# Lymphatus/caesium-clt

Measured on AMD Instinct MI355X. Metric: megapixels/sec JPEG q=80 1920x1080 batch, higher is better.
Workload: dtype int32

## Files before the change

### caesium-clt_amd/csrc/k_trellis.hip

```cpp
#include <algorithm>
#include <atomic>
#include <cassert>
#include <utility>

#include "kernels.h"

namespace csh {

#define CSH_TR_CAP 16
#define CSH_TR_WGU uint32_t(CSH_TR_WG)
#define CSH_TR_SPILL (63 - CSH_TR_CAP)
#define CSH_TR_MAXWG 2048
size_t trellis_spill_words(uint32_t nslots) { return size_t(nslots) * CSH_TR_SPILL * 3u * CSH_TR_WGU; }

#ifdef CSH_EMUL
#define CSH_ANY(p) (p)
#define CSH_WAVE_OR(v) (v)
#define CSH_SPILL_LD(ptr) (*(ptr))
#define CSH_SPILL_ST(ptr, v) (*(ptr) = (v))
#else
#define CSH_ANY(p) (__ballot(p) != 0ull)
__device__ __forceinline__ static unsigned tr_wave_or(unsigned v) {
    const unsigned n = 32u - unsigned(__clz(v));
    unsigned r = 0;
    if (__ballot(n >= 8u)) r = 8u;
    if (__ballot(n >= r + 4u)) r += 4u;
    if (__ballot(n >= r + 2u)) r += 2u;
    if (__ballot(n >= r + 1u)) r += 1u;
    return r ? 1u << (r - 1u) : 0u;
}
#define CSH_WAVE_OR(v) tr_wave_or(v)
#define CSH_SPILL_LD(ptr) __builtin_nontemporal_load(ptr)
#define CSH_SPILL_ST(ptr, v) __builtin_nontemporal_store((v), (ptr))
#endif

using Oct8 = std::integer_sequence<int, 0, 1, 2, 3, 4, 5, 6, 7>;
static constexpr uint8_t kN2Z[64] = {0,  1,  5,  6,  14, 15, 27, 28, 2,  4,  7,  13, 16, 26, 29, 42, 3,  8,  12, 17, 25, 30,
                                     41, 43, 9,  11, 18, 24, 31, 40, 44, 53, 10, 19, 23, 32, 39, 45, 52, 54, 20, 22, 33, 38,
                                     46, 51, 55, 60, 21, 34, 37, 47, 50, 56, 59, 61, 35, 36, 48, 49, 57, 58, 62, 63};
template <int I>
__device__ __forceinline__ static int tr_half(const uint4 &v) {
    uint32_t w = (I / 2 == 0) ? v.x : (I / 2 == 1) ? v.y : (I / 2 == 2) ? v.z : v.w;
    return (I & 1) ? (int(w) >> 16) : (int(w << 16) >> 16);
}
template <int J, int... I>
__device__ __forceinline__ static void tr_unpack(int r[64], const uint4 &v, std::integer_sequence<int, I...>) { ((r[8 * J + I] = tr_half<I>(v)), ...); }
template <int... J>
__device__ __forceinline__ static void tr_load(const int16_t *__restrict__ blk, int r[64], std::integer_sequence<int, J...>) {
    const uint4 v[8] = {*reinterpret_cast<const uint4 *>(blk + CSH_RAW_OCT * J)...};
    (tr_unpack<J>(r, v[J], Oct8()), ...);
}
__device__ __forceinline__ static int tr_level(int x, int d, uint32_t mul, uint32_t sh) {
    const uint32_t a = uint32_t(x + (d >> 1)) << sh;
    return int(uint32_t((uint64_t(a & 0xFFFFFFu) * uint64_t(mul & 0xFFFFFFu)) >> 32));
}
__device__ __forceinline__ static int tr_bitlen(unsigned v) { return 32 - __clz(v); }
__device__ __forceinline__ static float tr_bits_f(uint32_t u) { float f; memcpy(&f, &u, 4); return f; }
__device__ __forceinline__ static uint32_t tr_f_bits(float f) { uint32_t u; memcpy(&u, &f, 4); return u; }

#define TRELLIS_LAMBDA_C1 0x1.ae89f995ad3adp+14
#define TRELLIS_LAMBDA_C2 0x1.6a09e667f3bcdp+16
#define TRELLIS_MAX_LEVEL 1023

struct TrLds {
    float (*A)[CSH_TR_WG];
    float (*Z)[CSH_TR_WG];
    uint32_t (*P)[CSH_TR_WG];
    const float *lenf;
    const float *runf;
    int lenEOB;
    const int32_t *q8;
    const uint32_t *qmul, *qsh;
    const float *lt;
    const float *rcp;
};

__device__ __forceinline__ static void trellis_stage(const TrellisCtx &c, uint32_t wi, float *s_lenf, float *s_runf, int *s_eob, int32_t *s_q8, uint32_t *s_qmul, uint32_t *s_qsh, float *s_lt, float *s_rcp) {
    const TrellisWork &w = c.work[wi];
    const ImgDesc &im = c.imgs[w.image];
    const DevQuant &Q = c.quant[im.qt_out[w.comp]];
    const int tid = int(threadIdx.x);
    const uint8_t *size = c.tables[w.table_ac].size;
    for (int i = tid; i < 16 * 11; i += CSH_TR_WG) {
        const int r = i / 11, sz = i % 11 + 1, l = sz <= 10 ? size[(r << 4) | sz] : 0;
        s_lenf[i] = l ? float(l + sz) : 1e38f;
    }
    if (tid < 4) s_runf[tid] = tid == 0 ? 0.0f : (size[0xF0] ? float(tid * int(size[0xF0])) : 1e38f);
    if (tid == 0) *s_eob = size[0x00];
    if (tid < 64) { s_q8[tid] = Q.div[tid]; s_qmul[tid] = Q.mul[tid]; s_qsh[tid] = Q.sh[tid]; s_lt[tid] = Q.lt[tid]; s_rcp[tid] = Q.rcp[tid]; }
}

__device__ __forceinline__ static void trellis_block(const TrellisCtx &c, uint32_t wi, uint32_t j, uint32_t wg_slot, const TrLds &L) {
    const TrellisWork &w = c.work[wi];
    const ImgDesc &im = c.imgs[w.image];
    const CompGeom g = im.out[w.comp];
    const int tid = int(threadIdx.x);
    const uint32_t slot = j * CSH_TR_WGU + uint32_t(tid);
    if (slot >= w.nunits) return;
    const uint32_t u = c.perm ? c.perm[w.unit_base + slot] : slot;
    const int by = int(u) / g.real_bw, b = by * g.bw + (int(u) - by * g.real_bw);
    uint32_t *sp = c.spill + size_t(wg_slot) * (CSH_TR_SPILL * 3u * CSH_TR_WGU) + uint32_t(tid);

    int r[64];
    tr_load(c.raw + raw_index(g.tile_base - c.raw_tile0, b), r, Oct8());
    CSH_SCHED_FENCE();
    float norm = 0.0f;
    CSH_UNROLL
    for (int n = 1; n < 64; n++) { const float vf = float(r[kN2Z[n]]); norm = norm + vf * vf; }
    norm = float(double(norm) / 63.0);
    const float lambda = float(TRELLIS_LAMBDA_C1 / (TRELLIS_LAMBDA_C2 + double(norm)));
    c.dcrec[w.unit_base + u] = (uint64_t(tr_f_bits(lambda)) << 32) | (uint32_t(r[0]) & 0xFFFFu);
    CSH_SCHED_FENCE();
    if (c.debug & 1u) return;

    uint32_t ne = 0;
    float Zrun = 0.0f;
    CSH_UNROLL
    for (int k = 1; k < 64; k++) {
        const int v = r[k], x = v < 0 ? -v : v;
        const float xf = float(x);
        int qv = int(tr_f_bits(__builtin_fmaf(xf, L.rcp[k], 12582912.0f)) & 0xFFFFu);
        qv = qv > TRELLIS_MAX_LEVEL ? TRELLIS_MAX_LEVEL : qv;
        if (qv) {
            const uint32_t P = uint32_t(x) | (uint32_t(k) << 15) | (uint32_t(qv) << 21) | (v < 0 ? 0x80000000u : 0u);
            if (ne < CSH_TR_CAP) { L.Z[ne][tid] = Zrun; L.P[ne][tid] = P; }
            else { CSH_SPILL_ST(sp + ((ne - CSH_TR_CAP) * 3u + 1u) * CSH_TR_WGU, tr_f_bits(Zrun)); CSH_SPILL_ST(sp + ((ne - CSH_TR_CAP) * 3u + 2u) * CSH_TR_WGU, P); }
            ne++;
        }
        Zrun = ((xf * xf) * lambda) * L.lt[k] + Zrun;
    }
    const float Z63 = Zrun;
    CSH_SCHED_FENCE();

    const float lenEOBf = float(L.lenEOB);
    if (c.debug & 2u) ne = 0;
    for (uint32_t t = 0; CSH_ANY(t < ne); t++) {
        const bool on = t < ne;
        float Zp; uint32_t P;
        if (t < CSH_TR_CAP) { Zp = L.Z[t][tid]; P = L.P[t][tid]; }
        else { Zp = tr_bits_f(CSH_SPILL_LD(sp + ((t - CSH_TR_CAP) * 3u + 1u) * CSH_TR_WGU)); P = CSH_SPILL_LD(sp + ((t - CSH_TR_CAP) * 3u + 2u) * CSH_TR_WGU); }
        if (!on) { Zp = 0.0f; P = 0u; }
        const int x = int(P & 0x7FFFu), kpos = int((P >> 15) & 63u), qval = int((P >> 21) & 1023u);
        const int q8 = L.q8[kpos];
        const float ltk = L.lt[kpos];
        const int ncand = on ? tr_bitlen(unsigned(qval)) : 0;
        const int ncmax = tr_bitlen(CSH_WAVE_OR(on ? unsigned(qval) : 0u));
        float dist[10];
        CSH_UNROLL
        for (int kc = 0; kc < 10; kc++) {
            dist[kc] = 1e38f;
            if (kc >= ncmax) continue;
            const int cand = kc < ncand - 1 ? (2 << kc) - 1 : qval;
            const int delta = __mul24(cand, q8) - x;
            dist[kc] = kc < ncand ? (float(__mul24(delta, delta)) * lambda) * ltk : 1e38f;
        }
        float bestc = 1e38f;
        uint32_t bestsel = 0;
        auto from = [&](int jj, int posj, float Aj, float Zj) {
            const int zr = kpos - 1 - posj;
            const float runf = L.runf[(zr >> 4) & 3];
            const float *lf = L.lenf + 11 * (zr & 15);
            const float tj = (Zp - Zj) + Aj;
            const uint32_t sel0 = uint32_t(jj + 1) << 4;
            CSH_UNROLL
            for (int kc = 0; kc < 10; kc++) {
                if (kc >= ncmax) break;
                const float cost = ((lf[kc] + runf) + dist[kc]) + tj;
                const bool better = cost < bestc;
                bestc = better ? cost : bestc;
                bestsel = better ? (sel0 | uint32_t(kc)) : bestsel;
            }
        };
        from(-1, 0, 0.0f, 0.0f);
        const int t_lds = int(t) < CSH_TR_CAP ? int(t) : CSH_TR_CAP;
        if (ncmax <= 4) {
            auto batch = [&](auto KCV) {
                constexpr int KC = decltype(KCV)::value;
                for (int j0 = 0; j0 < t_lds; j0 += 4) {
                    uint32_t Pj[4]; float Aj[4], Zj[4];
                    CSH_UNROLL
                    for (int i = 0; i < 4; i++) { const int r = j0 + i < CSH_TR_CAP ? j0 + i : CSH_TR_CAP - 1; Pj[i] = L.P[r][tid]; Aj[i] = L.A[r][tid]; Zj[i] = L.Z[r][tid]; }
                    float cost[4][KC];
                    CSH_UNROLL
                    for (int i = 0; i < 4; i++) {
                        const int zr = kpos - 1 - int((Pj[i] >> 15) & 63u);
                        const float runf = L.runf[(zr >> 4) & 3];
                        const float *lf = L.lenf + 11 * (zr & 15);
                        const float tj = j0 + i < t_lds ? (Zp - Zj[i]) + Aj[i] : 1e38f;
                        CSH_UNROLL
                        for (int kc = 0; kc < KC; kc++) cost[i][kc] = ((lf[kc] + runf) + dist[kc]) + tj;
                    }
                    CSH_UNROLL
                    for (int i = 0; i < 4; i++) {
                        CSH_UNROLL
                        for (int kc = 0; kc < KC; kc++) {
                            const bool better = cost[i][kc] < bestc;
                            bestc = better ? cost[i][kc] : bestc;
                            bestsel = better ? ((uint32_t(j0 + i + 1) << 4) | uint32_t(kc)) : bestsel;
                        }
                    }
                }
            };
            if (ncmax <= 1) batch(std::integral_constant<int, 1>());
            else if (ncmax == 2) batch(std::integral_constant<int, 2>());
            else if (ncmax == 3) batch(std::integral_constant<int, 3>());
            else batch(std::integral_constant<int, 4>());
        } else
            for (int jj = 0; jj < t_lds; jj++) from(jj, int((L.P[jj][tid] >> 15) & 63u), L.A[jj][tid], L.Z[jj][tid]);
        for (int jj = CSH_TR_CAP; jj < int(t); jj++) {
            const uint32_t *q = sp + (uint32_t(jj - CSH_TR_CAP) * 3u) * CSH_TR_WGU;
            from(jj, int((CSH_SPILL_LD(q + 2 * CSH_TR_WG) >> 15) & 63u), tr_bits_f(CSH_SPILL_LD(q)), tr_bits_f(CSH_SPILL_LD(q + CSH_TR_WG)));
        }
        if (on) {
            const int bk = int(bestsel & 15u);
            const uint32_t level = uint32_t(bk < ncand - 1 ? (2 << bk) - 1 : qval);
            const float Zi = (float(__mul24(x, x)) * lambda) * ltk + Zp;
            const uint32_t P2 = (bestsel >> 4) | ((level == uint32_t(qval) && qval < TRELLIS_MAX_LEVEL) ? 0x4000u : 0u) | (uint32_t(kpos) << 15) | (level << 21) | (P & 0x80000000u);
            if (t < CSH_TR_CAP) { L.A[t][tid] = bestc; L.Z[t][tid] = Zi; L.P[t][tid] = P2; }
            else { uint32_t *q = sp + ((t - CSH_TR_CAP) * 3u) * CSH_TR_WGU; CSH_SPILL_ST(q, tr_f_bits(bestc)); CSH_SPILL_ST(q + CSH_TR_WG, tr_f_bits(Zi)); CSH_SPILL_ST(q + 2 * CSH_TR_WG, P2); }
        }
    }

    float best = Z63 + lenEOBf;
    int last = -1;
    for (uint32_t e = 0; CSH_ANY(e < ne); e++) {
        float Ae, Ze; uint32_t Pe;
        if (e < CSH_TR_CAP) { Ae = L.A[e][tid]; Ze = L.Z[e][tid]; Pe = L.P[e][tid]; }
        else { const uint32_t *q = sp + ((e - CSH_TR_CAP) * 3u) * CSH_TR_WGU; Ae = tr_bits_f(CSH_SPILL_LD(q)); Ze = tr_bits_f(CSH_SPILL_LD(q + CSH_TR_WG)); Pe = CSH_SPILL_LD(q + 2 * CSH_TR_WG); }
        float cost = (Ae + Z63) - Ze;
        if (int((Pe >> 15) & 63u) < 63) cost = cost + lenEOBf;
        if (e < ne && cost < best) { best = cost; last = int(e); }
    }

    if (c.debug & 4u) return;
    uint64_t kept = 0;
    for (int e = last; CSH_ANY(e >= 0);) {
        if (e >= 0) {
            uint32_t Pe;
            if (e < CSH_TR_CAP) Pe = L.P[e][tid]; else Pe = CSH_SPILL_LD(sp + (uint32_t(e - CSH_TR_CAP) * 3u + 2u) * CSH_TR_WGU);
            kept |= 1ull << e;
            e = int(Pe & 63u) - 1;
        }
    }
    const bool to_tile = !(c.ac_lists && w.ac_lists);
    int16_t *dst = to_tile ? c.coef + coef_index(g.tile_base, b, 0) : nullptr;
    uint32_t *lst = nullptr;
    if (c.nz_pool && w.nzset != 0xFFFFFFFFu) {
        const NzSet &S = c.nzsets[w.nzset];
        const NzList &L0 = c.nzlists[S.list[0]];
        const uint32_t rec = L0.chunk0 + (u >> 8);
        if (c.nz_chunk_cnt[rec]) lst = c.nz_pool + L0.base + c.nz_chunk_off[rec] + c.blk_off[w.unit_base + u];
    }
    uint32_t room = ne;
    if (lst && c.blk_cnt) {
        room = c.blk_cnt[w.unit_base + u];
#ifdef CSH_EMUL
        if (room != ne) { fprintf(stderr, "k_trellis_ac: block %u of unit %u has %u list entries but %u levels\n", u, w.unit_base, room, ne); abort(); }
#endif
    }
    for (uint32_t e0 = 0; CSH_ANY(e0 < ne); e0 += 4) {
        uint32_t ent[4] = {0u, 0u, 0u, 0u};
        CSH_UNROLL
        for (uint32_t i = 0; i < 4; i++) {
            const uint32_t e = e0 + i;
            if (e < ne) {
                uint32_t Pe;
                if (e < CSH_TR_CAP) Pe = L.P[e][tid]; else Pe = CSH_SPILL_LD(sp + ((e - CSH_TR_CAP) * 3u + 2u) * CSH_TR_WGU);
                const int pos = int((Pe >> 15) & 63u), level = ((kept >> e) & 1ull) ? int((Pe >> 21) & 1023u) : 0;
                if (to_tile && !(((kept >> e) & 1ull) && (Pe & 0x4000u))) dst[coef_off(pos)] = int16_t((Pe >> 31) ? -level : level);
                ent[i] = uint32_t(pos) | ((Pe >> 31) ? 128u : 0u) | (uint32_t(level) << 8) | ((u & 255u) << 23);
            }
        }
        if (lst && e0 < ne && e0 < room) {
            if (e0 + 4 <= ne && e0 + 4 <= room) {
#ifdef CSH_EMUL
                memcpy(lst + e0, ent, 16);
#else
                typedef uint32_t tr_u32x4_a4 __attribute__((ext_vector_type(4), aligned(4)));
                tr_u32x4_a4 v; v.x = ent[0]; v.y = ent[1]; v.z = ent[2]; v.w = ent[3];
                *reinterpret_cast<tr_u32x4_a4 *>(lst + e0) = v;
#endif
            } else {
                CSH_UNROLL
                for (uint32_t i = 0; i < 4; i++) if (e0 + i < ne && e0 + i < room) lst[e0 + i] = ent[i];
            }
        }
    }
}

__global__ void __launch_bounds__(256) k_trellis_sort(TrellisCtx c) {
    CSH_SHARED uint32_t s_cnt[64];
    const TrellisWork w = c.work[blockIdx.x];
    const uint8_t *cnt = c.blk_cnt + w.unit_base;
    uint32_t *perm = c.perm + w.unit_base;
    CSH_PHASE_LOOP(4) {
        if (phase == 0) { if (threadIdx.x < 64) s_cnt[threadIdx.x] = 0; continue; }
        if (phase == 1) { for (uint32_t u = threadIdx.x; u < w.nunits; u += 256) atomicAdd(&s_cnt[cnt[u] & 63u], 1u); continue; }
        if (phase == 2) {
            if (threadIdx.x == 0) { uint32_t at = 0; for (int k = 63; k >= 0; k--) { const uint32_t n = s_cnt[k]; s_cnt[k] = at; at += n; } }
            continue;
        }
        for (uint32_t u = threadIdx.x; u < w.nunits; u += 256) perm[atomicAdd(&s_cnt[cnt[u] & 63u], 1u)] = u;
    }
}
void launch_trellis_sort(hipStream_t st, const TrellisCtx &c) { if (c.nwork && c.perm && c.blk_cnt) CSH_LAUNCH_PHASED(k_trellis_sort, 4, dim3(unsigned(c.nwork)), dim3(256), st, c); }

__global__ void __launch_bounds__(CSH_TR_WG) k_trellis_ac(TrellisCtx c) {
    CSH_SHARED float s_A[CSH_TR_CAP][CSH_TR_WG];
    CSH_SHARED float s_Z[CSH_TR_CAP][CSH_TR_WG];
    CSH_SHARED uint32_t s_P[CSH_TR_CAP][CSH_TR_WG];
    CSH_SHARED float s_lenf[16 * 11 + 16];
    CSH_SHARED float s_runf[4];
    CSH_SHARED int s_eob;
    CSH_SHARED int32_t s_q8[64];
    CSH_SHARED uint32_t s_qmul[64];
    CSH_SHARED uint32_t s_qsh[64];
    CSH_SHARED float s_lt[64];
    CSH_SHARED float s_rcp[64];
    TrLds L; L.A = s_A; L.Z = s_Z; L.P = s_P; L.lenf = s_lenf; L.runf = s_runf; L.q8 = s_q8; L.qmul = s_qmul; L.qsh = s_qsh; L.lt = s_lt; L.rcp = s_rcp;
#ifdef CSH_EMUL
    CSH_PHASE_LOOP(2) {
        const TrellisRun rn = c.runs[blockIdx.x];
        if (phase == 0) { trellis_stage(c, rn.work, s_lenf, s_runf, &s_eob, s_q8, s_qmul, s_qsh, s_lt, s_rcp); continue; }
        L.lenEOB = s_eob;
        for (uint32_t j = rn.j; j < rn.j + rn.n; j++) trellis_block(c, rn.work, j, 0u, L);
    }
#else
    CSH_SHARED uint32_t s_run;
    for (;;) {
        if (threadIdx.x == 0) s_run = atomicAdd(c.queue, 1u);
        __syncthreads();
        const uint32_t ri = s_run;
        if (ri >= c.nruns) break;
        const TrellisRun rn = c.runs[ri];
        trellis_stage(c, rn.work, s_lenf, s_runf, &s_eob, s_q8, s_qmul, s_qsh, s_lt, s_rcp);
        __syncthreads();
        L.lenEOB = s_eob;
        for (uint32_t j = rn.j; j < rn.j + rn.n; j++) trellis_block(c, rn.work, j, blockIdx.x, L);
        __syncthreads();
    }
#endif
}

__device__ static const uint8_t kStdDcLen[2][12] = {{2, 3, 3, 3, 3, 3, 4, 5, 6, 7, 8, 9}, {2, 2, 2, 3, 4, 5, 6, 7, 8, 9, 10, 11}};

__global__ void __launch_bounds__(64) k_trellis_dc(TrellisCtx c) {
    const uint32_t ri = blockIdx.x * blockDim.x + threadIdx.x;
    if (ri >= c.nrows) return;
    const uint32_t rr = c.rows[ri];
    const TrellisWork w = c.work[rr >> 16];
    const ImgDesc &im = c.imgs[w.image];
    const CompGeom g = im.out[w.comp];
    const DevQuant &Q = c.quant[im.qt_out[w.comp]];
    const int row = int(rr & 0xFFFFu);
    int ncand = (2 + 60 / int(Q.q[0])) | 1;
    ncand = ncand > 9 ? 9 : ncand;
    CSH_SHARED float s_costs[64][13];
    float *s_cost = s_costs[threadIdx.x & 63u];
    for (int i = 0; i < 12; i++) s_cost[i] = float(i + int(w.table_dc < 0 ? kStdDcLen[w.comp ? 1 : 0][i] : c.tables[w.table_dc].size[i]));
    s_cost[12] = __builtin_inff();
    const int q = Q.div[0];
    const uint32_t qmul = Q.mul[0], qsh = Q.sh[0];
    const float lt0 = Q.lt[0];
    const int half = ncand / 2;
    int last_dc = 0;
    const int by1 = (row + 1) * g.v < g.real_bh ? (row + 1) * g.v : g.real_bh;
    for (int by = row * g.v; by < by1; by++) {
        float acc[9];
        int cprev[9];
        CSH_UNROLL
        for (int k = 0; k < 9; k++) { acc[k] = 0.0f; cprev[k] = 0; }
        int qprev = 0, sprev = 0;
        bool cprev_clamped = false;
        uint64_t rec_next = c.dcrec[w.unit_base + uint32_t(by * g.real_bw)];
        for (int bi = 0; bi < g.real_bw; bi++) {
            const uint32_t u = uint32_t(by * g.real_bw + bi);
            const uint64_t rec = rec_next;
            if (bi + 1 < g.real_bw) rec_next = c.dcrec[w.unit_base + u + 1u];
            const int raw0 = int(int16_t(uint16_t(rec & 0xFFFFu)));
            const float lambda_dc = tr_bits_f(uint32_t(rec >> 32)) * lt0;
            const int x = raw0 < 0 ? -raw0 : raw0;
            const int qval = tr_level(x, q, qmul, qsh);
            const int sgn = raw0 < 0 ? 1 : 0;
            const bool clamped = qval + half > TRELLIS_MAX_LEVEL;
            uint64_t bt = 0;
            float nacc[9];
            int ccur[9];
            float dist[9];
            CSH_UNROLL
            for (int k = 0; k < 9; k++) {
                int cand = qval - half + k;
                cand = cand > TRELLIS_MAX_LEVEL ? TRELLIS_MAX_LEVEL : cand;
                cand = cand < -TRELLIS_MAX_LEVEL ? -TRELLIS_MAX_LEVEL : cand;
                const int delta = k < ncand ? cand * q - x : 0;
                dist[k] = k < ncand ? float(delta * delta) * lambda_dc : __builtin_inff();
                ccur[k] = sgn ? -cand : cand;
            }
            if (bi == 0) {
                CSH_UNROLL
                for (int k = 0; k < 9; k++) { const int d = ccur[k] - last_dc, bits = tr_bitlen(unsigned(d < 0 ? -d : d)); nacc[k] = s_cost[bits] + dist[k]; }
            } else if (clamped || cprev_clamped) {
                CSH_UNROLL
                for (int k = 0; k < 9; k++) {
                    float bc = 0.0f;
                    uint32_t bl = 0;
                    CSH_UNROLL
                    for (int l = 0; l < 9; l++) {
                        const int d = ccur[k] - cprev[l], bits = tr_bitlen(unsigned(d < 0 ? -d : d));
                        const float cost = (s_cost[bits] + dist[k]) + acc[l];
                        if (l == 0 || cost < bc) { bc = cost; bl = uint32_t(l); }
                    }
                    nacc[k] = bc;
                    bt |= uint64_t(bl) << (4 * k);
                }
            } else {
                const bool same = sgn == sprev;
                const int base = same ? qval - qprev : qval + qprev - 2 * half;
                float cd[17];
                CSH_UNROLL
                for (int i = 0; i < 17; i++) { const int d = base + (i - 8); const int dd = same ? d : d + 8; cd[i] = s_cost[tr_bitlen(unsigned(dd < 0 ? -dd : dd))]; }
                CSH_UNROLL
                for (int k = 0; k < 9; k++) {
                    float bc = 0.0f;
                    uint32_t bl = 0;
                    CSH_UNROLL
                    for (int l = 0; l < 9; l++) {
                        const float cbits = same ? cd[k - l + 8] : cd[k + l];
                        const float cost = (cbits + dist[k]) + acc[l];
                        if (l == 0 || cost < bc) { bc = cost; bl = uint32_t(l); }
                    }
                    nacc[k] = bc;
                    bt |= uint64_t(bl) << (4 * k);
                }
            }
            CSH_UNROLL
            for (int k = 0; k < 9; k++) { acc[k] = nacc[k]; cprev[k] = ccur[k]; }
            qprev = qval; sprev = sgn; cprev_clamped = clamped;
            c.dcbt[w.unit_base + u] = bt | (uint64_t(uint32_t(qval)) << 36) | (uint64_t(raw0 < 0 ? 1u : 0u) << 47);
        }
        float bv = acc[0];
        uint32_t j = 0;
        CSH_UNROLL
        for (int i = 1; i < 9; i++) if (i < ncand && acc[i] < bv) { bv = acc[i]; j = uint32_t(i); }
        uint64_t bt_next = c.dcbt[w.unit_base + uint32_t(by * g.real_bw + g.real_bw - 1)];
        for (int bi = g.real_bw - 1; bi >= 0; bi--) {
            const uint64_t rec = bt_next;
            if (bi > 0) bt_next = c.dcbt[w.unit_base + uint32_t(by * g.real_bw + bi - 1)];
            int cand = int((rec >> 36) & 2047u) - half + int(j);
            cand = cand > TRELLIS_MAX_LEVEL ? TRELLIS_MAX_LEVEL : cand;
            cand = cand < -TRELLIS_MAX_LEVEL ? -TRELLIS_MAX_LEVEL : cand;
            cand = ((rec >> 47) & 1u) ? -cand : cand;
            c.coef[coef_index(g.tile_base, by * g.bw + bi, 0)] = int16_t(cand);
            if (bi == g.real_bw - 1) last_dc = cand;
            j = uint32_t((rec >> (4 * j)) & 15u);
        }
    }
}

#ifdef CSH_EMUL
uint32_t trellis_ac_slots() { return 1u; }
#else
uint32_t trellis_ac_slots() {
    static std::atomic<uint32_t> cached[64];
    int dev = 0;
    if (hipGetDevice(&dev) != hipSuccess) dev = 0;
    dev &= 63;
    uint32_t n = cached[dev].load(std::memory_order_relaxed);
    if (n) return n;
    int per_cu = 0, cus = 0;
    if (hipOccupancyMaxActiveBlocksPerMultiprocessor(&per_cu, k_trellis_ac, CSH_TR_WG, 0) != hipSuccess || per_cu < 1) per_cu = 1;
    if (hipDeviceGetAttribute(&cus, hipDeviceAttributeMultiprocessorCount, dev) != hipSuccess || cus < 1) cus = 1;
    n = uint32_t(per_cu) * uint32_t(cus);
    n = n < CSH_TR_MAXWG ? n : CSH_TR_MAXWG;
    cached[dev].store(n, std::memory_order_relaxed);
    return n;
}
#endif

void launch_trellis_ac(hipStream_t st, const TrellisCtx &c) {
    if (!c.nruns || !c.nslots) return;
#ifdef CSH_EMUL
    assert(c.nslots >= 1u);
    CSH_LAUNCH_PHASED(k_trellis_ac, 2, dim3(c.nruns), dim3(CSH_TR_WG), st, c);
#else
    const uint32_t nwg = std::min(std::min(c.nruns, c.nslots), trellis_ac_slots());
    CSH_LAUNCH(k_trellis_ac, dim3(nwg), dim3(CSH_TR_WG), st, c);
#endif
}
void launch_trellis_dc(hipStream_t st, const TrellisCtx &c) {
    if (c.nrows) CSH_LAUNCH(k_trellis_dc, dim3((c.nrows + 63) / 64), dim3(64), st, c);
}

}
```

Baseline: 45330.

## Precompute combined run+size rate table and fold EOB search into trellis pass

Replaces the separate per-run length table and ZRL run-cost table with a single 64x11 LDS table indexed directly by position distance, so each candidate cost needs one LDS load and one fewer add and index computation. The final pass that rescans all nonzero states to find the best EOB point is merged into the main trellis loop, which avoids rereading A/Z/P from LDS and spill memory. Unused qmul/qsh staging is dropped and the batch clamp now uses t_lds. The trade-off is a larger LDS table filled once per run, plus a changed dummy P value for inactive lanes.

After: 45390, median of 4. No clear change (+0.1%).

```diff
diff --git a/caesium-clt_amd/csrc/k_trellis.hip b/caesium-clt_amd/csrc/k_trellis.hip
--- a/caesium-clt_amd/csrc/k_trellis.hip
+++ b/caesium-clt_amd/csrc/k_trellis.hip
@@ -62,32 +62,38 @@
 #define TRELLIS_LAMBDA_C2 0x1.6a09e667f3bcdp+16
 #define TRELLIS_MAX_LEVEL 1023
 
+__device__ __forceinline__ static const float *tr_rate_row(const float *rate, int kpos, int posj) {
+#ifdef CSH_EMUL
+    if (unsigned(kpos - posj) > 63u) { fprintf(stderr, "k_trellis_ac: rate row %d (position %d behind %d)\n", kpos - posj, kpos, posj); abort(); }
+#endif
+    return rate + 11 * (kpos - posj);
+}
+
 struct TrLds {
     float (*A)[CSH_TR_WG];
     float (*Z)[CSH_TR_WG];
     uint32_t (*P)[CSH_TR_WG];
-    const float *lenf;
-    const float *runf;
+    const float *rate;
     int lenEOB;
     const int32_t *q8;
-    const uint32_t *qmul, *qsh;
     const float *lt;
     const float *rcp;
 };
 
-__device__ __forceinline__ static void trellis_stage(const TrellisCtx &c, uint32_t wi, float *s_lenf, float *s_runf, int *s_eob, int32_t *s_q8, uint32_t *s_qmul, uint32_t *s_qsh, float *s_lt, float *s_rcp) {
+__device__ __forceinline__ static void trellis_stage(const TrellisCtx &c, uint32_t wi, float *s_rate, int *s_eob, int32_t *s_q8, float *s_lt, float *s_rcp) {
     const TrellisWork &w = c.work[wi];
     const ImgDesc &im = c.imgs[w.image];
     const DevQuant &Q = c.quant[im.qt_out[w.comp]];
     const int tid = int(threadIdx.x);
     const uint8_t *size = c.tables[w.table_ac].size;
-    for (int i = tid; i < 16 * 11; i += CSH_TR_WG) {
-        const int r = i / 11, sz = i % 11 + 1, l = sz <= 10 ? size[(r << 4) | sz] : 0;
-        s_lenf[i] = l ? float(l + sz) : 1e38f;
-    }
-    if (tid < 4) s_runf[tid] = tid == 0 ? 0.0f : (size[0xF0] ? float(tid * int(size[0xF0])) : 1e38f);
+    for (int i = tid; i < 64 * 11; i += CSH_TR_WG) {
+        const int zr = i / 11 - 1, sz = i % 11 + 1, l = (zr >= 0 && sz <= 10) ? size[((zr & 15) << 4) | sz] : 0;
+        const float lenf = l ? float(l + sz) : 1e38f;
+        const float runf = zr < 16 ? 0.0f : (size[0xF0] ? float((zr >> 4) * int(size[0xF0])) : 1e38f);
+        s_rate[i] = lenf + runf;
+    }
     if (tid == 0) *s_eob = size[0x00];
-    if (tid < 64) { s_q8[tid] = Q.div[tid]; s_qmul[tid] = Q.mul[tid]; s_qsh[tid] = Q.sh[tid]; s_lt[tid] = Q.lt[tid]; s_rcp[tid] = Q.rcp[tid]; }
+    if (tid < 64) { s_q8[tid] = Q.div[tid]; s_lt[tid] = Q.lt[tid]; s_rcp[tid] = Q.rcp[tid]; }
 }
 
 __device__ __forceinline__ static void trellis_block(const TrellisCtx &c, uint32_t wi, uint32_t j, uint32_t wg_slot, const TrLds &L) {
@@ -134,12 +140,14 @@
 
     const float lenEOBf = float(L.lenEOB);
     if (c.debug & 2u) ne = 0;
+    float best = Z63 + lenEOBf;
+    int last = -1;
     for (uint32_t t = 0; CSH_ANY(t < ne); t++) {
         const bool on = t < ne;
         float Zp; uint32_t P;
         if (t < CSH_TR_CAP) { Zp = L.Z[t][tid]; P = L.P[t][tid]; }
         else { Zp = tr_bits_f(CSH_SPILL_LD(sp + ((t - CSH_TR_CAP) * 3u + 1u) * CSH_TR_WGU)); P = CSH_SPILL_LD(sp + ((t - CSH_TR_CAP) * 3u + 2u) * CSH_TR_WGU); }
-        if (!on) { Zp = 0.0f; P = 0u; }
+        if (!on) { Zp = 0.0f; P = 63u << 15; }
         const int x = int(P & 0x7FFFu), kpos = int((P >> 15) & 63u), qval = int((P >> 21) & 1023u);
         const int q8 = L.q8[kpos];
         const float ltk = L.lt[kpos];
@@ -157,15 +165,13 @@
         float bestc = 1e38f;
         uint32_t bestsel = 0;
         auto from = [&](int jj, int posj, float Aj, float Zj) {
-            const int zr = kpos - 1 - posj;
-            const float runf = L.runf[(zr >> 4) & 3];
-            const float *lf = L.lenf + 11 * (zr & 15);
+            const float *lf = tr_rate_row(L.rate, kpos, posj);
             const float tj = (Zp - Zj) + Aj;
             const uint32_t sel0 = uint32_t(jj + 1) << 4;
             CSH_UNROLL
             for (int kc = 0; kc < 10; kc++) {
                 if (kc >= ncmax) break;
-                const float cost = ((lf[kc] + runf) + dist[kc]) + tj;
+                const float cost = (lf[kc] + dist[kc]) + tj;
                 const bool better = cost < bestc;
                 bestc = better ? cost : bestc;
                 bestsel = better ? (sel0 | uint32_t(kc)) : bestsel;
@@ -179,16 +185,14 @@
                 for (int j0 = 0; j0 < t_lds; j0 += 4) {
                     uint32_t Pj[4]; float Aj[4], Zj[4];
                     CSH_UNROLL
-                    for (int i = 0; i < 4; i++) { const int r = j0 + i < CSH_TR_CAP ? j0 + i : CSH_TR_CAP - 1; Pj[i] = L.P[r][tid]; Aj[i] = L.A[r][tid]; Zj[i] = L.Z[r][tid]; }
+                    for (int i = 0; i < 4; i++) { const int r = j0 + i < t_lds ? j0 + i : t_lds - 1; Pj[i] = L.P[r][tid]; Aj[i] = L.A[r][tid]; Zj[i] = L.Z[r][tid]; }
                     float cost[4][KC];
                     CSH_UNROLL
                     for (int i = 0; i < 4; i++) {
-                        const int zr = kpos - 1 - int((Pj[i] >> 15) & 63u);
-                        const float runf = L.runf[(zr >> 4) & 3];
-                        const float *lf = L.lenf + 11 * (zr & 15);
+                        const float *lf = tr_rate_row(L.rate, kpos, int((Pj[i] >> 15) & 63u));
                         const float tj = j0 + i < t_lds ? (Zp - Zj[i]) + Aj[i] : 1e38f;
                         CSH_UNROLL
-                        for (int kc = 0; kc < KC; kc++) cost[i][kc] = ((lf[kc] + runf) + dist[kc]) + tj;
+                        for (int kc = 0; kc < KC; kc++) cost[i][kc] = (lf[kc] + dist[kc]) + tj;
                     }
                     CSH_UNROLL
                     for (int i = 0; i < 4; i++) {
@@ -218,18 +222,10 @@
             const uint32_t P2 = (bestsel >> 4) | ((level == uint32_t(qval) && qval < TRELLIS_MAX_LEVEL) ? 0x4000u : 0u) | (uint32_t(kpos) << 15) | (level << 21) | (P & 0x80000000u);
             if (t < CSH_TR_CAP) { L.A[t][tid] = bestc; L.Z[t][tid] = Zi; L.P[t][tid] = P2; }
             else { uint32_t *q = sp + ((t - CSH_TR_CAP) * 3u) * CSH_TR_WGU; CSH_SPILL_ST(q, tr_f_bits(bestc)); CSH_SPILL_ST(q + CSH_TR_WG, tr_f_bits(Zi)); CSH_SPILL_ST(q + 2 * CSH_TR_WG, P2); }
-        }
-    }
-
-    float best = Z63 + lenEOBf;
-    int last = -1;
-    for (uint32_t e = 0; CSH_ANY(e < ne); e++) {
-        float Ae, Ze; uint32_t Pe;
-        if (e < CSH_TR_CAP) { Ae = L.A[e][tid]; Ze = L.Z[e][tid]; Pe = L.P[e][tid]; }
-        else { const uint32_t *q = sp + ((e - CSH_TR_CAP) * 3u) * CSH_TR_WGU; Ae = tr_bits_f(CSH_SPILL_LD(q)); Ze = tr_bits_f(CSH_SPILL_LD(q + CSH_TR_WG)); Pe = CSH_SPILL_LD(q + 2 * CSH_TR_WG); }
-        float cost = (Ae + Z63) - Ze;
-        if (int((Pe >> 15) & 63u) < 63) cost = cost + lenEOBf;
-        if (e < ne && cost < best) { best = cost; last = int(e); }
+            float cost = (bestc + Z63) - Zi;
+            if (kpos < 63) cost = cost + lenEOBf;
+            if (cost < best) { best = cost; last = int(t); }
+        }
     }
 
     if (c.debug & 4u) return;
@@ -309,19 +305,16 @@
     CSH_SHARED float s_A[CSH_TR_CAP][CSH_TR_WG];
     CSH_SHARED float s_Z[CSH_TR_CAP][CSH_TR_WG];
     CSH_SHARED uint32_t s_P[CSH_TR_CAP][CSH_TR_WG];
-    CSH_SHARED float s_lenf[16 * 11 + 16];
-    CSH_SHARED float s_runf[4];
+    CSH_SHARED float s_rate[64 * 11];
     CSH_SHARED int s_eob;
     CSH_SHARED int32_t s_q8[64];
-    CSH_SHARED uint32_t s_qmul[64];
-    CSH_SHARED uint32_t s_qsh[64];
     CSH_SHARED float s_lt[64];
     CSH_SHARED float s_rcp[64];
-    TrLds L; L.A = s_A; L.Z = s_Z; L.P = s_P; L.lenf = s_lenf; L.runf = s_runf; L.q8 = s_q8; L.qmul = s_qmul; L.qsh = s_qsh; L.lt = s_lt; L.rcp = s_rcp;
+    TrLds L; L.A = s_A; L.Z = s_Z; L.P = s_P; L.rate = s_rate; L.q8 = s_q8; L.lt = s_lt; L.rcp = s_rcp;
 #ifdef CSH_EMUL
     CSH_PHASE_LOOP(2) {
         const TrellisRun rn = c.runs[blockIdx.x];
-        if (phase == 0) { trellis_stage(c, rn.work, s_lenf, s_runf, &s_eob, s_q8, s_qmul, s_qsh, s_lt, s_rcp); continue; }
+        if (phase == 0) { trellis_stage(c, rn.work, s_rate, &s_eob, s_q8, s_lt, s_rcp); continue; }
         L.lenEOB = s_eob;
         for (uint32_t j = rn.j; j < rn.j + rn.n; j++) trellis_block(c, rn.work, j, 0u, L);
     }
@@ -333,7 +326,7 @@
         const uint32_t ri = s_run;
         if (ri >= c.nruns) break;
         const TrellisRun rn = c.runs[ri];
-        trellis_stage(c, rn.work, s_lenf, s_runf, &s_eob, s_q8, s_qmul, s_qsh, s_lt, s_rcp);
+        trellis_stage(c, rn.work, s_rate, &s_eob, s_q8, s_lt, s_rcp);
         __syncthreads();
         L.lenEOB = s_eob;
         for (uint32_t j = rn.j; j < rn.j + rn.n; j++) trellis_block(c, rn.work, j, blockIdx.x, L);
```
